# TritonDataCenter/node-cueball

Hardware: AMD Instinct MI355X
Metric: pool claims/sec (8-backend synthetic TCP set) (higher is better)
Workload: dtype n/a; 1 GPU; model=ConnectionPool claim/release (config: headline), global_batch=20000, seq_len=1, parallelism=1 worker processes (event loops), backends=8, spares=8, maximum=16, concurrency=16

## Files before the change

cueball_amd/_native/speed.cpp:

```cpp

#define PY_SSIZE_T_CLEAN
#include <Python.h>
#include <structmember.h>
#include <cmath>
#include <cstring>
#include <ctime>

#include "lathist.h"

#ifndef CUEBALL_HANDLE_HOOKS
#define CUEBALL_HANDLE_HOOKS 1
#endif
#ifndef CUEBALL_SLOT_HOOKS
#define CUEBALL_SLOT_HOOKS 1
#endif
#ifndef CUEBALL_LAZY_SCOPES
#define CUEBALL_LAZY_SCOPES 1
#endif
#ifndef CUEBALL_VECTORCALL
#define CUEBALL_VECTORCALL 1
#endif
#ifndef CUEBALL_EXACT_TYPES
#define CUEBALL_EXACT_TYPES 1
#endif
#ifndef CUEBALL_VALID_IDENTITY
#define CUEBALL_VALID_IDENTITY 1
#endif
#if !defined(Py_TPFLAGS_HAVE_VECTORCALL) && defined(_Py_TPFLAGS_HAVE_VECTORCALL)
#define Py_TPFLAGS_HAVE_VECTORCALL _Py_TPFLAGS_HAVE_VECTORCALL
#endif

namespace {

PyObject *s_stateChanged;
PyObject *s_listener;
PyObject *s_on;
PyObject *s_remove_listener;
PyObject *s_call_soon;
PyObject *s_call_later;
PyObject *s_cancel;
PyObject *s_state_prefix;
PyObject *s_dot;
PyObject *s_underscore;
PyObject *s_flush_name;
PyObject *s_internal;
PyObject *s_is_closed;

PyObject *g_get_loop;
PyObject *g_fsm_error;
PyObject *g_entry_name_cache;
PyObject *g_flush_batches;
PyObject *g_tracer;
PyObject *g_remove_desc;

static inline PyObject *
resolve_loop(PyObject *loop)
{
    if (loop != NULL && loop != Py_None) {
        Py_INCREF(loop);
        return loop;
    }
    return PyObject_CallOneArg(g_get_loop, Py_None);
}


typedef struct {
    PyObject_HEAD
    PyObject *ev_events;
    PyObject *ev_dict;
    PyObject *ev_weakrefs;
    unsigned long ev_gen;
    unsigned long ev_lk_gen;
    long ev_lk_cnt[4];
    Py_ssize_t ev_lk_len[4];
    int ev_lk_ok;
} Emitter;

extern PyTypeObject EmitterType;
extern PyTypeObject ConnErrCbType;
extern PyTypeObject KitCbType;

static inline int
listener_is_own_internal(PyObject *listener)
{
    PyTypeObject *tp = Py_TYPE(listener);
    return tp == &ConnErrCbType || tp == &KitCbType;
}

#define SMALL_LIST_KEEP 8

static inline int
list_append_keep(PyObject *ls, PyObject *item)
{
    PyListObject *l = (PyListObject *)ls;
    Py_ssize_t n = Py_SIZE(l);
    if (n < l->allocated) {
        Py_INCREF(item);
        l->ob_item[n] = item;
        Py_SET_SIZE(l, n + 1);
        return 0;
    }
    return PyList_Append(ls, item);
}

static inline int
list_remove_at_keep(PyObject *ls, Py_ssize_t i)
{
    PyListObject *l = (PyListObject *)ls;
    Py_ssize_t n = Py_SIZE(l);
    if (l->allocated > SMALL_LIST_KEEP)
        return PyList_SetSlice(ls, i, i + 1, NULL);
    PyObject *item = l->ob_item[i];
    for (Py_ssize_t j = i; j + 1 < n; j++)
        l->ob_item[j] = l->ob_item[j + 1];
    Py_SET_SIZE(l, n - 1);
    Py_DECREF(item);
    return 0;
}

int
Emitter_init(PyObject *self_, PyObject *args, PyObject *kwds)
{
    Emitter *self = (Emitter *)self_;
    (void)args; (void)kwds;
    if (self->ev_events == NULL) {
        self->ev_events = PyDict_New();
        if (self->ev_events == NULL)
            return -1;
    }
    return 0;
}

int
Emitter_traverse(PyObject *self_, visitproc visit, void *arg)
{
    Emitter *self = (Emitter *)self_;
    Py_VISIT(self->ev_events);
    Py_VISIT(self->ev_dict);
    return 0;
}

int
Emitter_clear_(PyObject *self_)
{
    Emitter *self = (Emitter *)self_;
    Py_CLEAR(self->ev_events);
    Py_CLEAR(self->ev_dict);
    return 0;
}

void
Emitter_dealloc(PyObject *self_)
{
    Emitter *self = (Emitter *)self_;
    PyTypeObject *tp = Py_TYPE(self_);
    PyObject_GC_UnTrack(self_);
    if (self->ev_weakrefs != NULL)
        PyObject_ClearWeakRefs(self_);
    Emitter_clear_(self_);
    tp->tp_free(self_);
}

PyObject *
emitter_add(Emitter *self, PyObject *event, PyObject *listener)
{
    if (self->ev_events == NULL) {
        self->ev_events = PyDict_New();
        if (self->ev_events == NULL)
            return NULL;
    }
    PyObject *ls = PyDict_GetItemWithError(self->ev_events, event);
    if (ls == NULL) {
        if (PyErr_Occurred())
            return NULL;
        ls = PyList_New(0);
        if (ls == NULL)
            return NULL;
        if (PyDict_SetItem(self->ev_events, event, ls) < 0) {
            Py_DECREF(ls);
            return NULL;
        }
        Py_DECREF(ls);
    }
    if (list_append_keep(ls, listener) < 0)
        return NULL;
    if (!listener_is_own_internal(listener))
        self->ev_gen++;
    Py_INCREF(listener);
    return listener;
}

PyObject *
Emitter_on(PyObject *self_, PyObject *const *args, Py_ssize_t nargs)
{
    if (nargs != 2) {
        PyErr_SetString(PyExc_TypeError, "on(event, listener)");
        return NULL;
    }
    return emitter_add((Emitter *)self_, args[0], args[1]);
}

typedef struct {
    PyObject_HEAD
    PyObject *ow_emitter;
    PyObject *ow_event;
    PyObject *ow_listener;
} OnceWrapper;

extern PyTypeObject OnceWrapperType;

PyObject *
OnceWrapper_call(PyObject *self_, PyObject *args, PyObject *kwds)
{
    OnceWrapper *self = (OnceWrapper *)self_;
    (void)kwds;
    PyObject *res = PyObject_CallMethodObjArgs(
        self->ow_emitter, s_remove_listener, self->ow_event,
        (PyObject *)self, NULL);
    if (res == NULL)
        return NULL;
    Py_DECREF(res);
    return PyObject_Call(self->ow_listener, args, NULL);
}

PyObject *
OnceWrapper_get_listener(PyObject *self_, void *closure)
{
    OnceWrapper *self = (OnceWrapper *)self_;
// ... 694 lines not shown
    return 0;
}

int
Scope_clear_(PyObject *self_)
{
    Scope *self = (Scope *)self_;
    Py_CLEAR(self->sc_fsm);
    Py_CLEAR(self->sc_listeners);
    Py_CLEAR(self->sc_timers);
    int nreg = self->sc_nreg;
    self->sc_nreg = 0;
    for (int i = 0; i < 3 * nreg; i++)
        Py_CLEAR(self->sc_reg[i]);
    return 0;
}

void
Scope_dealloc(PyObject *self_)
{
    PyObject_GC_UnTrack(self_);
    Scope_clear_(self_);
    if (scope_freelist_n < SCOPE_FREELIST_MAX)
        scope_freelist[scope_freelist_n++] = (Scope *)self_;
    else
        PyObject_GC_Del(self_);
}

PyMethodDef Scope_methods[] = {
    {"on", (PyCFunction)(void (*)(void))Scope_on, METH_FASTCALL, NULL},
    {"timeout", (PyCFunction)(void (*)(void))Scope_timeout, METH_FASTCALL,
     NULL},
    {"interval", (PyCFunction)(void (*)(void))Scope_interval,
     METH_FASTCALL, NULL},
    {"immediate", Scope_immediate, METH_O, NULL},
    {"callback", Scope_callback, METH_O, NULL},
    {"valid_transitions", Scope_valid_transitions, METH_O, NULL},
    {"goto_state", Scope_goto_state, METH_O, NULL},
    {"_dispose", Scope_dispose, METH_NOARGS, NULL},
    {NULL, NULL, 0, NULL},
};

PyGetSetDef Scope_getset[] = {
    {(char *)"active", Scope_get_active, NULL, NULL, NULL},
    {NULL, NULL, NULL, NULL, NULL},
};

PyTypeObject ScopeType = {
    PyVarObject_HEAD_INIT(NULL, 0)
    "cueball_amd._speed.StateScope",
    sizeof(Scope),
    0,
    Scope_dealloc,
    0, 0, 0, 0, 0, 0, 0, 0, 0, 0, 0, 0, 0, 0,
    Py_TPFLAGS_DEFAULT | Py_TPFLAGS_HAVE_GC,
    "FSM state scope (native)",
    Scope_traverse,
    Scope_clear_,
    0, 0, 0, 0,
    Scope_methods,
    0,
    Scope_getset,
};


struct FSMOb {
    Emitter base;
    PyObject *f_loop;
    PyObject *f_state;
    PyObject *f_scope;
    PyObject *f_valid;
    PyObject *f_pending;
    PyObject **f_eq;
    Py_ssize_t f_eq_head, f_eq_len, f_eq_cap;
    PyObject *f_eq_inl[4];
    PyObject *f_hist[8];
    unsigned long f_hist_n;
    PyObject *f_flush_bound;
    PyObject *f_fastkit;
    PyObject *f_watchkit;
    PyObject *f_ctx;
    int f_entering;
    int f_emit_scheduled;
};

int slotkit_maybe_entry(PyObject *kit_, FSMOb *fsm, PyObject *target);
int slotkit_smgr_hook(PyObject *kit_, PyObject *st, unsigned long serial);
unsigned long slotkit_slot_serial(PyObject *kit_);
int ch_emit_state_changed(FSMOb *self, PyObject *st);

static inline Scope *
fsm_need_scope(FSMOb *self)
{
    if (self->f_scope == NULL)
        self->f_scope = (PyObject *)scope_new((PyObject *)self);
    return (Scope *)self->f_scope;
}

extern PyObject *t_empty;
extern PyTypeObject CHType;
extern PyTypeObject CTType;
void ch_terminal_cleanup(FSMOb *self);

typedef PyObject *(*ch_entry_fn)(PyObject *, PyObject *);
ch_entry_fn ch_direct_entry(FSMOb *self, PyObject *target);

extern PyTypeObject FSMType;
extern PyTypeObject SlotBaseType;

PyTypeObject *g_handle_cls;
PyTypeObject *g_slot_cls;
PyTypeObject *g_pool_cls;

static inline int
is_handle(PyObject *x)
{
#if CUEBALL_EXACT_TYPES
    if (Py_TYPE(x) == g_handle_cls)
        return 1;
#endif
    return PyObject_TypeCheck(x, &CHType);
}

static inline int
is_slot(PyObject *x)
{
#if CUEBALL_EXACT_TYPES
    if (Py_TYPE(x) == g_slot_cls)
        return 1;
#endif
    return PyObject_TypeCheck(x, &SlotBaseType);
}

static inline int
is_fsm(PyObject *x)
{
#if CUEBALL_EXACT_TYPES
    PyTypeObject *tp = Py_TYPE(x);
    if (tp == g_pool_cls || tp == g_slot_cls || tp == g_handle_cls)
        return 1;
#endif
    return PyObject_TypeCheck(x, &FSMType);
}

PyObject *
fsm_get_loop_of(FSMOb *fsm)
{
    return fsm->f_loop;
}

#define FSM_EQ_INLINE 4
#define FSM_HISTORY 8

static void
fsm_eq_compact(FSMOb *f)
{
    if (f->f_eq_head == 0)
        return;
    Py_ssize_t n = f->f_eq_len - f->f_eq_head;
    memmove(f->f_eq, f->f_eq + f->f_eq_head, n * sizeof(PyObject *));
    f->f_eq_head = 0;
    f->f_eq_len = n;
}

static int
fsm_eq_push(FSMOb *f, PyObject *st)
{
    if (f->f_eq == NULL) {
        f->f_eq = f->f_eq_inl;
        f->f_eq_cap = FSM_EQ_INLINE;
        f->f_eq_head = f->f_eq_len = 0;
    }
    if (f->f_eq_len == f->f_eq_cap) {
        if (f->f_eq_head > 0) {
            fsm_eq_compact(f);
        } else {
            Py_ssize_t ncap = f->f_eq_cap * 2;
            PyObject **items;
            if (f->f_eq == f->f_eq_inl) {
                items = (PyObject **)PyMem_Malloc(
                    ncap * sizeof(PyObject *));
                if (items != NULL)
                    memcpy(items, f->f_eq_inl, sizeof(f->f_eq_inl));
            } else {
                items = (PyObject **)PyMem_Realloc(
// ... 234 lines not shown
            Py_DECREF(fb);
            return -1;
        }
        Py_DECREF(h);
        batch = (PyObject *)fb;
        Py_DECREF(fb);
    }
    if (PyList_Append(((FlushBatch *)batch)->fb_list,
                      (PyObject *)self) < 0)
        return -1;
    return 0;
}

PyObject *
entry_attr_name(PyObject *state)
{
    PyObject *name = PyDict_GetItemWithError(g_entry_name_cache, state);
    if (name != NULL) {
        Py_INCREF(name);
        return name;
    }
    if (PyErr_Occurred())
        return NULL;
    PyObject *replaced = PyObject_CallMethod(state, "replace", "OO",
                                             s_dot, s_underscore);
    if (replaced == NULL)
        return NULL;
    name = PyUnicode_Concat(s_state_prefix, replaced);
    Py_DECREF(replaced);
    if (name == NULL)
        return NULL;
    PyUnicode_InternInPlace(&name);
    if (PyDict_SetItem(g_entry_name_cache, state, name) < 0) {
        Py_DECREF(name);
        return NULL;
    }
    return name;
}

int
check_valid(FSMOb *self, PyObject *from, PyObject *state)
{
    if (self->f_valid == NULL)
        return 0;
#if CUEBALL_VALID_IDENTITY
    if (PyTuple_CheckExact(self->f_valid)) {
        PyObject *v = self->f_valid;
        for (Py_ssize_t i = 0, n = PyTuple_GET_SIZE(v); i < n; i++)
            if (PyTuple_GET_ITEM(v, i) == state)
                return 0;
    }
#endif
    int c = PySequence_Contains(self->f_valid, state);
    if (c < 0)
        return -1;
    if (!c) {
        PyErr_Format(g_fsm_error,
                     "%s: invalid transition %R -> %R (valid: %R)",
                     Py_TYPE(self)->tp_name,
                     from ? from : Py_None, state, self->f_valid);
        return -1;
    }
    return 0;
}

int
fsm_enter_loop(FSMOb *self, PyObject *state)
{
    PyObject *next_state = state;
    Py_INCREF(next_state);
    while (next_state != NULL) {
        PyObject *target = next_state;
        next_state = NULL;
        if (self->f_scope != NULL) {
            PyObject *old = self->f_scope;
            self->f_scope = NULL;
            PyObject *r = Scope_dispose(old, NULL);
            Py_DECREF(old);
            if (r == NULL) {
                Py_DECREF(target);
                return -1;
            }
            Py_DECREF(r);
        }
        Py_CLEAR(self->f_valid);
        Py_INCREF(target);
        Py_XSETREF(self->f_state, target);
        Py_INCREF(target);
        Py_XSETREF(self->f_hist[self->f_hist_n % FSM_HISTORY], target);
        self->f_hist_n++;
#if !CUEBALL_LAZY_SCOPES
        if (fsm_need_scope(self) == NULL) {
            Py_DECREF(target);
            return -1;
        }
#endif

        if (g_tracer != NULL && g_tracer != Py_None) {
            PyObject *targs[2] = {(PyObject *)self, target};
            PyObject *tr = PyObject_Vectorcall(g_tracer, targs, 2, NULL);
            if (tr == NULL) {
                Py_DECREF(target);
                return -1;
            }
            Py_DECREF(tr);
        }

        int handled = 0;
        if (self->f_fastkit != NULL) {
            self->f_entering = 1;
            handled = slotkit_maybe_entry(self->f_fastkit, self, target);
            self->f_entering = 0;
            if (handled < 0) {
                Py_DECREF(target);
                return -1;
            }
        }
        PyObject *r;
        ch_entry_fn direct = handled ? NULL : ch_direct_entry(self, target);
        if (handled) {
            r = Py_None;
            Py_INCREF(r);
        } else if (direct != NULL) {
            self->f_entering = 1;
            r = direct((PyObject *)self, NULL);
            self->f_entering = 0;
        } else {
            PyObject *attr = entry_attr_name(target);
            if (attr == NULL) {
                Py_DECREF(target);
                return -1;
            }
            PyObject *entry = PyObject_GetAttr((PyObject *)self, attr);
            Py_DECREF(attr);
            if (entry == NULL) {
                PyErr_Clear();
                PyErr_Format(g_fsm_error,
                             "%s has no state-entry function for %R",
                             Py_TYPE(self)->tp_name, target);
                Py_DECREF(target);
                return -1;
            }
            PyObject *scope = (PyObject *)fsm_need_scope(self);
            if (scope == NULL) {
                Py_DECREF(entry);
                Py_DECREF(target);
                return -1;
            }
            Py_INCREF(scope);
            self->f_entering = 1;
            r = PyObject_CallOneArg(entry, scope);
            Py_DECREF(entry);
            Py_DECREF(scope);
            self->f_entering = 0;
        }
        PyObject *pend = self->f_pending;
        self->f_pending = NULL;
        if (r == NULL) {
            Py_XDECREF(pend);
            Py_DECREF(target);
            return -1;
        }
        Py_DECREF(r);
        if (fsm_queue_state_changed(self, target) < 0) {
            Py_XDECREF(pend);
            Py_DECREF(target);
// ... 901 lines not shown
};

static void
latency_types_init(void)
{
    LatHistType.tp_flags = Py_TPFLAGS_DEFAULT;
    LatHistType.tp_methods = LatHist_methods;
    LatHistType.tp_getset = LatHist_getset;
    LatHistType.tp_new = LatHist_new;

    PoolLatType.tp_dealloc = PoolLat_dealloc;
    PoolLatType.tp_flags = Py_TPFLAGS_DEFAULT | Py_TPFLAGS_HAVE_GC;
    PoolLatType.tp_traverse = PoolLat_traverse;
    PoolLatType.tp_clear = PoolLat_clear_;
    PoolLatType.tp_members = PoolLat_members;
    PoolLatType.tp_new = PoolLat_new;
}


PyObject *g_err_claim_timeout;
PyObject *g_err_cueball;
PyObject *g_err_misused;
PyObject *g_capture_stack;

PyObject *s_claim;
PyObject *s_warn;
PyObject *s_incr;
PyObject *s_claim_timeout_evt;
PyObject *s_is_in_state;
PyObject *s_time;
PyObject *s_waiting, *s_claiming, *s_claimed, *s_released, *s_closed,
         *s_cancelled, *s_failed, *s_idle, *s_error_evt;
PyObject *t_waiting_valid;
PyObject *t_claiming_valid;
PyObject *t_claimed_valid;
PyObject *t_empty;
PyObject *s_leak_events[4];

int g_stack_on = 1;
PyObject *g_stack_placeholder;
PyObject *g_inf;

static inline PyObject *
capture_stack(void)
{
    if (!g_stack_on && g_stack_placeholder != NULL) {
        Py_INCREF(g_stack_placeholder);
        return g_stack_placeholder;
    }
    return PyObject_CallNoArgs(g_capture_stack);
}

extern PyObject *s_busy_st;
PyObject *slotkit_conn_err_cb(PyObject *slot, PyObject *handle);

struct NQueue;
typedef struct {
    PyObject_HEAD
    struct NQueue *pc_idleq;
    struct NQueue *pc_waiters;
    struct NQueue *pc_initq;
    PyObject *pc_counters;
    PyObject *pc_dead;
    PoolLatOb *pc_lat;
    PyObject *pc_log;
    int pc_no_codel;
} PoolCtx;

extern PyTypeObject PoolCtxType;
PoolCtx *pool_ctx(PyObject *pool);
PoolCtx *pool_ctx_private(PoolCtx *base, PoolLatOb *lat, PyObject *log);

typedef struct {
    FSMOb base;
    PyObject *chb_pool;
    PyObject *chb_claim_stack;
    PyObject *chb_callback;
    PyObject *chb_slot;
    PyObject *chb_release_stack;
    PyObject *chb_connection;
    PyObject *chb_last_error;
    PyObject *chb_waiter_node;
    PoolCtx *chb_ctx;
    double chb_claim_timeout;
    double chb_started;
    double chb_claimed_at;
    int chb_pre[4];
    unsigned char chb_have_pre;
    unsigned char chb_throw_error;
    unsigned char chb_cancelled;
    unsigned char chb_leak_check;
    unsigned char chb_pinger;
    unsigned char chb_lat_open;
    unsigned char chb_tk_on;
    unsigned char chb_tk_err_on_empty;
    unsigned long chb_bk_serial;
    Py_ssize_t chb_bk_pos;
} CHOb;

extern PyTypeObject CHType;

static inline PoolLatOb *
ch_lat(CHOb *h)
{
    return h->chb_ctx != NULL ? h->chb_ctx->pc_lat : NULL;
}

static inline PyObject *
ch_log(CHOb *h)
{
    return h->chb_ctx != NULL && h->chb_ctx->pc_log != NULL
        ? h->chb_ctx->pc_log : Py_None;
}

long
c_count_listeners(PyObject *emitter, PyObject *event)
{
    if (!PyObject_TypeCheck(emitter, &EmitterType))
        return -2;
    Emitter *em = (Emitter *)emitter;
    if (em->ev_events == NULL)
        return 0;
    PyObject *ls = PyDict_GetItemWithError(em->ev_events, event);
    if (ls == NULL)
        return PyErr_Occurred() ? -1 : 0;
    long count = 0;
    Py_ssize_t n = PyList_GET_SIZE(ls);
    for (Py_ssize_t i = 0; i < n; i++) {
        PyObject *h = PyList_GET_ITEM(ls, i);
        if (!PyCallable_Check(h))
            continue;
        PyObject *marker = NULL;
        if (_PyObject_LookupAttr(h, s_internal, &marker) < 0)
            return -1;
        if (marker != NULL) {
            int truthy = PyObject_IsTrue(marker);
            Py_DECREF(marker);
            if (truthy < 0)
                return -1;
            if (truthy)
                continue;
        }
        PyObject *target = NULL;
        if (Py_TYPE(h) == &OnceWrapperType) {
            target = ((OnceWrapper *)h)->ow_listener;
            Py_INCREF(target);
        } else if (_PyObject_LookupAttr(h, s_listener, &target) < 0) {
            return -1;
        }
        if (target != NULL && target != h) {
            if (_PyObject_LookupAttr(target, s_internal, &marker) < 0) {
                Py_DECREF(target);
                return -1;
            }
            if (marker != NULL) {
                int truthy = PyObject_IsTrue(marker);
                Py_DECREF(marker);
                if (truthy < 0) {
                    Py_DECREF(target);
                    return -1;
                }
                if (truthy) {
                    Py_DECREF(target);
                    continue;
                }
            }
        }
        Py_XDECREF(target);
        count++;
    }
    return count;
}

int
emitter_leak_counts(PyObject *conn, long out[4])
{
    if (!PyObject_TypeCheck(conn, &EmitterType))
        return -2;
    Emitter *em = (Emitter *)conn;
    Py_ssize_t lens[4];
    for (int i = 0; i < 4; i++) {
        PyObject *ls = NULL;
        if (em->ev_events != NULL) {
            ls = PyDict_GetItemWithError(em->ev_events, s_leak_events[i]);
            if (ls == NULL && PyErr_Occurred())
                return -1;
        }
        lens[i] = (ls != NULL && PyList_Check(ls)) ? PyList_GET_SIZE(ls)
                                                   : -1;
    }
    if (em->ev_lk_ok && em->ev_lk_gen == em->ev_gen &&
        memcmp(lens, em->ev_lk_len, sizeof(lens)) == 0) {
        memcpy(out, em->ev_lk_cnt, sizeof(em->ev_lk_cnt));
        return 0;
    }
    unsigned long gen = em->ev_gen;
    for (int i = 0; i < 4; i++) {
        long c = c_count_listeners(conn, s_leak_events[i]);
        if (c < 0)
            return -1;
        out[i] = c;
    }
    em->ev_lk_ok = 0;
    if (gen == em->ev_gen) {
        memcpy(em->ev_lk_cnt, out, sizeof(em->ev_lk_cnt));
        memcpy(em->ev_lk_len, lens, sizeof(lens));
        em->ev_lk_gen = gen;
        em->ev_lk_ok = 1;
    }
    return 0;
}

typedef struct {
    PyObject_HEAD
    PyObject *ce_handle;
} ConnErrCb;

extern PyTypeObject ConnErrCbType;

PyObject *conn_err_fire(CHOb *h, PyObject *err);

PyObject *
ConnErrCb_call(PyObject *self_, PyObject *args, PyObject *kwds)
{
    CHOb *h = (CHOb *)((ConnErrCb *)self_)->ce_handle;
    (void)kwds;
    PyObject *err = (PyTuple_GET_SIZE(args) > 0)
        ? PyTuple_GET_ITEM(args, 0) : Py_None;
    return conn_err_fire(h, err);
}

PyObject *
conn_err_fire(CHOb *h, PyObject *err)
{
    long cnt = c_count_listeners(h->chb_connection, s_error_evt);
    if (cnt == -1)
        return NULL;
    if (cnt == 0 && h->chb_throw_error) {
        if (PyExceptionInstance_Check(err)) {
            PyErr_SetObject((PyObject *)Py_TYPE(err), err);
        } else {
            PyErr_SetObject(PyExc_RuntimeError, err);
        }
        return NULL;
    }
    PyObject *msg = PyUnicode_FromString(
        "connection emitted error while claimed");
    if (msg == NULL)
        return NULL;
    PyObject *r = PyObject_CallMethodObjArgs(ch_log(h), s_warn, msg,
                                             NULL);
    Py_DECREF(msg);
    if (r == NULL)
        return NULL;
    Py_DECREF(r);
    PyObject *evt = PyUnicode_FromString("error-while-claimed");
    if (evt == NULL)
        return NULL;
    r = PyObject_CallMethodObjArgs(h->chb_pool, s_incr, evt, NULL);
    Py_DECREF(evt);
    if (r == NULL)
        return NULL;
    Py_DECREF(r);
    Py_RETURN_NONE;
}

int
ConnErrCb_traverse(PyObject *self_, visitproc visit, void *arg)
{
    Py_VISIT(((ConnErrCb *)self_)->ce_handle);
    return 0;
}

int
ConnErrCb_clear_(PyObject *self_)
{
    Py_CLEAR(((ConnErrCb *)self_)->ce_handle);
    return 0;
}

void
ConnErrCb_dealloc(PyObject *self_)
{
    PyObject_GC_UnTrack(self_);
    ConnErrCb_clear_(self_);
    PyObject_GC_Del(self_);
}

PyObject *
ConnErrCb_get_internal(PyObject *self_, void *closure)
{
    (void)self_; (void)closure;
    Py_RETURN_TRUE;
// ... 290 lines not shown
        if (cb == NULL) {
            Py_DECREF(ms);
            return NULL;
        }
        PyObject *args[2] = {ms, cb};
        PyObject *r = Scope_timeout(scope, args, 2);
        Py_DECREF(ms);
        Py_DECREF(cb);
        if (r == NULL)
            return NULL;
        Py_DECREF(r);
    }
    Py_RETURN_NONE;
}

PyObject *
CH_state_claiming(PyObject *self_, PyObject *scope)
{
    CHOb *self = (CHOb *)self_;
    (void)scope;
    Py_INCREF(t_claiming_valid);
    Py_XSETREF(self->base.f_valid, t_claiming_valid);
    PyObject *slot = self->chb_slot;
    if (slot != NULL && is_slot(slot) &&
        ((FSMOb *)slot)->f_fastkit != NULL) {
        FSMOb *sf = (FSMOb *)slot;
        PyObject *fs = sf->f_state;
        if (!(fs == s_idle ||
              (fs != NULL && PyUnicode_Compare(fs, s_idle) == 0))) {
            PyErr_SetString(g_fsm_error, "claim only in idle");
            return NULL;
        }
        if (slot_field_set(&((SlotOb *)slot)->sl_handle)) {
            PyErr_SetString(g_fsm_error, "slot already has a handle");
            return NULL;
        }
        slot_field_store(&((SlotOb *)slot)->sl_handle, self_);
        if (fsm_goto_state(sf, s_busy_st) < 0)
            return NULL;
        Py_RETURN_NONE;
    }
    PyObject *r = PyObject_CallMethodObjArgs(slot, s_claim,
                                             self_, NULL);
    if (r == NULL)
        return NULL;
    Py_DECREF(r);
    Py_RETURN_NONE;
}

PyObject *
CH_state_claimed(PyObject *self_, PyObject *scope)
{
    CHOb *self = (CHOb *)self_;
    Py_INCREF(t_claimed_valid);
    Py_XSETREF(self->base.f_valid, t_claimed_valid);

    if (self->chb_cancelled) {
        if (fsm_goto_state(&self->base, s_released) < 0)
            return NULL;
        Py_RETURN_NONE;
    }

    PyObject *conn = self->chb_connection;
    long pre[4] = {0, 0, 0, 0};
    int lk = emitter_leak_counts(conn, pre);
    if (lk == -1)
        return NULL;
    for (int i = 0; i < 4; i++)
        self->chb_pre[i] = lk == -2 ? 0 : (int)pre[i];
    self->chb_have_pre = 1;

    PyObject *ec = slotkit_conn_err_cb(self->chb_slot, self_);
    if (ec != NULL) {
        Py_INCREF(ec);
    } else {
        ConnErrCb *nec = PyObject_GC_New(ConnErrCb, &ConnErrCbType);
        if (nec == NULL)
            return NULL;
        Py_INCREF(self_);
        nec->ce_handle = self_;
        PyObject_GC_Track((PyObject *)nec);
        ec = (PyObject *)nec;
    }
    if (scope == NULL)
        scope = (PyObject *)fsm_need_scope(&self->base);
    if (scope == NULL) {
        Py_DECREF(ec);
        return NULL;
    }
    PyObject *args[3] = {conn, s_error_evt, ec};
    PyObject *r = Scope_on(scope, args, 3);
    Py_DECREF(ec);
    if (r == NULL)
        return NULL;
    Py_DECREF(r);

    PoolLatOb *lat = ch_lat(self);
    if (lat != NULL && !self->chb_pinger) {
        int err = 0;
        double now = poollat_now_ms(lat, &err);
        if (err)
            return NULL;
        lat->pl_wait->h.record_ms(now - self->chb_started);
        self->chb_claimed_at = now;
        self->chb_lat_open = 1;
    }

    PyObject *cbargs[3] = {Py_None, self_, conn};
    r = PyObject_Vectorcall(self->chb_callback, cbargs, 3, NULL);
    if (r == NULL)
        return NULL;
    Py_DECREF(r);
    Py_RETURN_NONE;
}

static int
ch_record_hold(CHOb *self)
{
    if (!self->chb_lat_open)
        return 0;
    self->chb_lat_open = 0;
    PoolLatOb *lat = ch_lat(self);
    if (lat == NULL)
        return 0;
    int err = 0;
    double now = poollat_now_ms(lat, &err);
    if (err)
        return -1;
    lat->pl_hold->h.record_ms(now - self->chb_claimed_at);
    return 0;
}

PyObject *
CH_state_released(PyObject *self_, PyObject *scope)
{
    CHOb *self = (CHOb *)self_;
    (void)scope;
    Py_INCREF(t_empty);
    Py_XSETREF(self->base.f_valid, t_empty);
    if (ch_record_hold(self) < 0)
        return NULL;
    if (!self->chb_leak_check || !self->chb_have_pre)
        Py_RETURN_NONE;
    PyObject *conn = self->chb_connection;
    long after[4];
    int lk = emitter_leak_counts(conn, after);
    if (lk == -1)
        return NULL;
    if (lk == -2)
        Py_RETURN_NONE;
    for (int i = 0; i < 4; i++) {
        long c = after[i];
        if (c > (long)self->chb_pre[i]) {
            PyObject *msg = PyUnicode_FromFormat(
                "connection claimer looks like it leaked event handlers "
                "(event=%S before=%ld after=%ld)",
                s_leak_events[i], (long)self->chb_pre[i], c);
            if (msg == NULL)
                return NULL;
            PyObject *r = PyObject_CallMethodObjArgs(ch_log(self), s_warn,
                                                     msg, NULL);
            Py_DECREF(msg);
            if (r == NULL)
                return NULL;
            Py_DECREF(r);
        }
    }
    Py_RETURN_NONE;
}

PyObject *
CH_state_closed(PyObject *self_, PyObject *scope)
{
    CHOb *self = (CHOb *)self_;
    (void)scope;
    Py_INCREF(t_empty);
    Py_XSETREF(self->base.f_valid, t_empty);
    if (ch_record_hold(self) < 0)
        return NULL;
    Py_RETURN_NONE;
}

PyObject *
CH_state_cancelled(PyObject *self_, PyObject *scope)
{
    CHOb *self = (CHOb *)self_;
    (void)scope;
    Py_INCREF(t_empty);
    Py_XSETREF(self->base.f_valid, t_empty);
    Py_RETURN_NONE;
}

PyObject *
CH_state_failed(PyObject *self_, PyObject *scope)
{
    CHOb *self = (CHOb *)self_;
// ... 24 lines not shown
    PyObject *err = PyObject_CallNoArgs(g_err_misused);
    if (err == NULL)
        return NULL;
    PyErr_SetObject(g_err_misused, err);
    Py_DECREF(err);
    return NULL;
}

PyObject *
CH_on(PyObject *self_, PyObject *const *args, Py_ssize_t nargs)
{
    if (nargs >= 1 && PyUnicode_Check(args[0])) {
        if (PyUnicode_CompareWithASCIIString(args[0], "readable") == 0 ||
            PyUnicode_CompareWithASCIIString(args[0], "close") == 0) {
            PyObject *err = PyObject_CallNoArgs(g_err_misused);
            if (err == NULL)
                return NULL;
            PyErr_SetObject(g_err_misused, err);
            Py_DECREF(err);
            return NULL;
        }
    }
    return Emitter_on(self_, args, nargs);
}

PyObject *
CH_once(PyObject *self_, PyObject *const *args, Py_ssize_t nargs)
{
    if (nargs >= 1 && PyUnicode_Check(args[0])) {
        if (PyUnicode_CompareWithASCIIString(args[0], "readable") == 0 ||
            PyUnicode_CompareWithASCIIString(args[0], "close") == 0) {
            PyObject *err = PyObject_CallNoArgs(g_err_misused);
            if (err == NULL)
                return NULL;
            PyErr_SetObject(g_err_misused, err);
            Py_DECREF(err);
            return NULL;
        }
    }
    return Emitter_once(self_, args, nargs);
}

PyObject *
CH_remove_listener(PyObject *self_, PyObject *const *args, Py_ssize_t nargs)
{
    CHOb *self = (CHOb *)self_;
    if (nargs != 2) {
        PyErr_SetString(PyExc_TypeError, "remove_listener(event, listener)");
        return NULL;
    }
    Py_ssize_t at;
    if (emitter_remove_core(&self->base.base, args, &at) < 0)
        return NULL;
    if (at >= 0 && at < self->chb_bk_pos &&
        (args[0] == s_stateChanged ||
         (PyUnicode_Check(args[0]) &&
          PyUnicode_Compare(args[0], s_stateChanged) == 0)))
        self->chb_bk_pos--;
    Py_RETURN_NONE;
}

PyObject *
CH_remove_all_listeners(PyObject *self_, PyObject *const *args,
                        Py_ssize_t nargs)
{
    ((CHOb *)self_)->chb_bk_pos = 0;
    return Emitter_remove_all_listeners(self_, args, nargs);
}


int
CH_traverse(PyObject *self_, visitproc visit, void *arg)
{
    CHOb *self = (CHOb *)self_;
    Py_VISIT(self->chb_pool);
    Py_VISIT(self->chb_claim_stack);
    Py_VISIT(self->chb_callback);
    Py_VISIT(self->chb_slot);
    Py_VISIT(self->chb_release_stack);
    Py_VISIT(self->chb_connection);
    Py_VISIT(self->chb_last_error);
    Py_VISIT(self->chb_waiter_node);
    Py_VISIT((PyObject *)self->chb_ctx);
    return FSM_traverse(self_, visit, arg);
}

int
CH_clear_(PyObject *self_)
{
    CHOb *self = (CHOb *)self_;
    Py_CLEAR(self->chb_pool);
    Py_CLEAR(self->chb_claim_stack);
    Py_CLEAR(self->chb_callback);
    Py_CLEAR(self->chb_slot);
    Py_CLEAR(self->chb_release_stack);
    Py_CLEAR(self->chb_connection);
    Py_CLEAR(self->chb_last_error);
    Py_CLEAR(self->chb_waiter_node);
    Py_CLEAR(self->chb_ctx);
    return FSM_clear_(self_);
}

void
CH_dealloc(PyObject *self_)
{
    CHOb *self = (CHOb *)self_;
    PyTypeObject *tp = Py_TYPE(self_);
    PyObject_GC_UnTrack(self_);
    if (self->base.base.ev_weakrefs != NULL)
        PyObject_ClearWeakRefs(self_);
    CH_clear_(self_);
    tp->tp_free(self_);
}

PyObject *
CH__setup(PyObject *self_, PyObject *const *args, Py_ssize_t nargs)
{
    CHOb *self = (CHOb *)self_;
    if (nargs != 7) {
        PyErr_SetString(PyExc_TypeError,
            "_setup(pool, stack, cb, log, timeout, throw_error, loop)");
        return NULL;
    }
    Py_INCREF(args[0]); Py_XSETREF(self->chb_pool, args[0]);
    Py_INCREF(args[1]); Py_XSETREF(self->chb_claim_stack, args[1]);
    Py_INCREF(args[2]); Py_XSETREF(self->chb_callback, args[2]);
    self->chb_claim_timeout = PyFloat_AsDouble(args[4]);
    if (self->chb_claim_timeout == -1.0 && PyErr_Occurred())
        return NULL;
    int throw_error = PyObject_IsTrue(args[5]);
    if (throw_error < 0)
        return NULL;
    self->chb_throw_error = throw_error;
    self->chb_cancelled = 0;
    self->chb_leak_check = 1;
    self->chb_pinger = 0;
    self->chb_have_pre = 0;
    self->chb_lat_open = 0;
    PoolCtx *cx = pool_ctx(args[0]);
    if (cx != NULL && cx->pc_log == args[3]) {
        Py_INCREF((PyObject *)cx);
    } else {
        PyObject *lat = NULL;
        if (cx != NULL) {
            lat = (PyObject *)cx->pc_lat;
            Py_XINCREF(lat);
        } else {
            if (_PyObject_LookupAttr(args[0], s_p_lat, &lat) < 0)
                return NULL;
            if (lat != NULL && Py_TYPE(lat) != &PoolLatType)
                Py_CLEAR(lat);
        }
        cx = pool_ctx_private(cx, (PoolLatOb *)lat, args[3]);
        Py_XDECREF(lat);
        if (cx == NULL)
            return NULL;
    }
    Py_XSETREF(self->chb_ctx, cx);

    PyObject *resolved = resolve_loop(args[6]);
    if (resolved == NULL)
        return NULL;
    Py_XSETREF(self->base.f_loop, resolved);
#if !CUEBALL_HANDLE_HOOKS
    if (Emitter_init(self_, NULL, NULL) < 0)
        return NULL;
#endif
    self->chb_tk_on = 0;
    self->chb_bk_serial = 0;
    if (fsm_goto_state(&self->base, s_waiting) < 0)
        return NULL;
    PoolLatOb *plat = ch_lat(self);
    if (plat != NULL && plat->pl_direct &&
        plat->pl_loop == self->base.f_loop) {
        int err = 0;
        self->chb_started = poollat_now_ms(plat, &err);
        if (err)
            return NULL;
        Py_RETURN_NONE;
    }
    PyObject *t = PyObject_CallMethodObjArgs(self->base.f_loop, s_time,
                                             NULL);
// ... 2743 lines not shown
static void
claim_method_type_init(void)
{
    ClaimMethodType.tp_dealloc = ClaimMethod_dealloc;
    ClaimMethodType.tp_vectorcall_offset =
        offsetof(ClaimMethod, cm_vectorcall);
    ClaimMethodType.tp_call = PyVectorcall_Call;
    ClaimMethodType.tp_flags = Py_TPFLAGS_DEFAULT | Py_TPFLAGS_HAVE_GC |
        Py_TPFLAGS_HAVE_VECTORCALL | Py_TPFLAGS_METHOD_DESCRIPTOR;
    ClaimMethodType.tp_traverse = ClaimMethod_traverse;
    ClaimMethodType.tp_clear = ClaimMethod_clear_;
    ClaimMethodType.tp_members = ClaimMethod_members;
    ClaimMethodType.tp_descr_get = ClaimMethod_descr_get;
}

static PyObject *
speed_claim_method(PyObject *mod, PyObject *const *args, Py_ssize_t nargs)
{
    (void)mod;
    if (nargs != 2 || !PyCallable_Check(args[0]) || !PyType_Check(args[1]) ||
        !PyType_IsSubtype((PyTypeObject *)args[1], &CHType)) {
        PyErr_SetString(PyExc_TypeError,
                        "claim_method(func, ClaimHandleBase subclass)");
        return NULL;
    }
#if !CUEBALL_VECTORCALL
    Py_INCREF(args[0]);
    return args[0];
#else
    ClaimMethod *cm = PyObject_GC_New(ClaimMethod, &ClaimMethodType);
    if (cm == NULL)
        return NULL;
    Py_INCREF(args[0]);
    cm->cm_func = args[0];
    Py_INCREF(args[1]);
    cm->cm_handle_cls = args[1];
    cm->cm_vectorcall = ClaimMethod_vectorcall;
    cm->cm_doc = PyObject_GetAttrString(args[0], "__doc__");
    cm->cm_name = PyObject_GetAttrString(args[0], "__name__");
    cm->cm_qualname = PyObject_GetAttrString(args[0], "__qualname__");
    cm->cm_module = PyObject_GetAttrString(args[0], "__module__");
    PyErr_Clear();
    PyObject_GC_Track((PyObject *)cm);
    return (PyObject *)cm;
#endif
}

static PyObject *
speed_set_cycle_classes(PyObject *mod, PyObject *const *args,
                        Py_ssize_t nargs)
{
    (void)mod;
    if (nargs != 3) {
        PyErr_SetString(PyExc_TypeError,
                        "_set_cycle_classes(handle_cls, slot_cls, pool_cls)");
        return NULL;
    }
    PyTypeObject *bases[3] = {&CHType, &SlotBaseType, &FSMType};
    PyTypeObject **dst[3] = {&g_handle_cls, &g_slot_cls, &g_pool_cls};
    for (int i = 0; i < 3; i++) {
        if (args[i] == Py_None)
            continue;
        PyTypeObject *cls = (PyTypeObject *)args[i];
        if (!PyType_Check(args[i]) || !PyType_IsSubtype(cls, bases[i]) ||
            (i > 0 && PyType_IsSubtype(cls, &CHType)) ||
            (i == 2 && PyType_IsSubtype(cls, &SlotBaseType))) {
            PyErr_SetString(PyExc_TypeError,
                "_set_cycle_classes: a ClaimHandleBase, a SlotBase and a "
                "plain FSM subclass required");
            return NULL;
        }
    }
    for (int i = 0; i < 3; i++) {
        if (args[i] == Py_None)
            continue;
        Py_INCREF(args[i]);
        PyTypeObject *old = *dst[i];
        *dst[i] = (PyTypeObject *)args[i];
        Py_XDECREF((PyObject *)old);
    }
    Py_RETURN_NONE;
}

PyObject *
speed_set_tracer(PyObject *mod, PyObject *fn)
{
    (void)mod;
    if (fn == Py_None) {
        Py_CLEAR(g_tracer);
    } else {
        Py_INCREF(fn);
        Py_XSETREF(g_tracer, fn);
    }
    Py_RETURN_NONE;
}

PyMethodDef speed_methods[] = {
    {"_set_claim_helpers",
     (PyCFunction)(void (*)(void))speed_set_claim_helpers, METH_FASTCALL,
     NULL},
    {"_set_tracer", speed_set_tracer, METH_O, NULL},
    {"_set_stack_traces",
     (PyCFunction)(void (*)(void))speed_set_stack_traces, METH_FASTCALL,
     NULL},
    {"count_listeners",
     (PyCFunction)(void (*)(void))speed_count_listeners, METH_FASTCALL,
     NULL},
    {"_set_helpers", (PyCFunction)(void (*)(void))speed_set_helpers,
     METH_FASTCALL, NULL},
    {"claim_fast", (PyCFunction)(void (*)(void))speed_claim_fast,
     METH_FASTCALL, NULL},
    {"pool_claim", (PyCFunction)(void (*)(void))speed_pool_claim,
     METH_FASTCALL, NULL},
    {"claim_method", (PyCFunction)(void (*)(void))speed_claim_method,
     METH_FASTCALL, NULL},
    {"_set_cycle_classes",
     (PyCFunction)(void (*)(void))speed_set_cycle_classes, METH_FASTCALL,
     NULL},
    {NULL, NULL, 0, NULL},
};

struct PyModuleDef speedmodule = {
    PyModuleDef_HEAD_INIT,
    "cueball_amd._speed",
    "Native event/FSM runtime core",
    -1,
    speed_methods,
};

}

PyMODINIT_FUNC
PyInit__speed(void)
{
    s_stateChanged = PyUnicode_InternFromString("stateChanged");
    s_listener = PyUnicode_InternFromString("listener");
    s_on = PyUnicode_InternFromString("on");
    s_remove_listener = PyUnicode_InternFromString("remove_listener");
    s_call_soon = PyUnicode_InternFromString("call_soon");
    s_call_later = PyUnicode_InternFromString("call_later");
    s_cancel = PyUnicode_InternFromString("cancel");
    s_state_prefix = PyUnicode_InternFromString("state_");
    s_dot = PyUnicode_InternFromString(".");
    s_underscore = PyUnicode_InternFromString("_");
    s_flush_name = PyUnicode_InternFromString("_flush_state_changed");
    s_internal = PyUnicode_InternFromString("_cueball_internal");
    s_is_closed = PyUnicode_InternFromString("is_closed");
    s_claim = PyUnicode_InternFromString("claim");
    s_warn = PyUnicode_InternFromString("warn");
    s_incr = PyUnicode_InternFromString("_incr_counter");
    s_claim_timeout_evt = PyUnicode_InternFromString("claim-timeout");
    s_is_in_state = PyUnicode_InternFromString("is_in_state");
    s_time = PyUnicode_InternFromString("time");
    s_waiting = PyUnicode_InternFromString("waiting");
    s_claiming = PyUnicode_InternFromString("claiming");
    s_claimed = PyUnicode_InternFromString("claimed");
    s_released = PyUnicode_InternFromString("released");
    s_closed = PyUnicode_InternFromString("closed");
    s_cancelled = PyUnicode_InternFromString("cancelled");
    s_failed = PyUnicode_InternFromString("failed");
    s_idle = PyUnicode_InternFromString("idle");
    s_error_evt = PyUnicode_InternFromString("error");
    t_waiting_valid = PyTuple_Pack(3, s_claiming, s_cancelled, s_failed);
    t_claiming_valid = PyTuple_Pack(3, s_claimed, s_waiting, s_cancelled);
    t_claimed_valid = PyTuple_Pack(2, s_released, s_closed);
    t_empty = PyTuple_New(0);
    s_leak_events[0] = PyUnicode_InternFromString("close");
    s_leak_events[1] = s_error_evt;
    s_leak_events[2] = PyUnicode_InternFromString("readable");
    s_leak_events[3] = PyUnicode_InternFromString("data");
    g_entry_name_cache = PyDict_New();
    if (g_entry_name_cache == NULL)
        return NULL;
    g_flush_batches = PyDict_New();
    if (g_flush_batches == NULL)
        return NULL;

    s_running_st = PyUnicode_InternFromString("running");
    s_p_idleq_node = PyUnicode_InternFromString("p_idleq_node");
    s_p_total_conns = PyUnicode_InternFromString("p_total_conns");
    s_p_busy_hwm = PyUnicode_InternFromString("p_busy_hwm");
    s_p_demand_hwm = PyUnicode_InternFromString("p_demand_hwm");
    s_ticket_slow = PyUnicode_InternFromString("_ticket_slow");
    s_p_idleq = PyUnicode_InternFromString("p_idleq");
    s_p_waiters = PyUnicode_InternFromString("p_waiters");
    s_p_initq = PyUnicode_InternFromString("p_initq");
    s_p_counters = PyUnicode_InternFromString("p_counters");
    s_p_rebal_scheduled = PyUnicode_InternFromString("p_rebal_scheduled");
    s_max_claim_queue = PyUnicode_InternFromString("max-claim-queue");
    s_queued_claim = PyUnicode_InternFromString("queued-claim");
    s_connected_st = PyUnicode_InternFromString("connected");
    s_busy_st = PyUnicode_InternFromString("busy");
    s_stopping_st = PyUnicode_InternFromString("stopping");
    s_stopped_st = PyUnicode_InternFromString("stopped");
    s_retrying_st = PyUnicode_InternFromString("retrying");
    s_connecting_st = PyUnicode_InternFromString("connecting");
    s_killing_st = PyUnicode_InternFromString("killing");
    s_unwanted_evt = PyUnicode_InternFromString("unwanted");
    s_sm_socket = PyUnicode_InternFromString("sm_socket");
    t_busy_valid = PyTuple_Pack(6, s_idle, s_stopping_st, s_stopped_st,
// ... 96 lines not shown
```

Baseline: 871,300 claims/s.

## Cache leak-listener counts by dict version tag and register conn error handler directly

Moves the per-emitter leak-count cache into a separately allocated struct that also holds the listener lists and the events dict's version tag. This lets a cache hit skip the four dict lookups when the dict is unchanged. Separately, the claim handle registers its connection 'error' listener directly on the connection instead of lazily creating a Scope, and unregisters it on the next state transition. The aim is to avoid scope allocation and disposal per claim, at the cost of more complex lifetime bookkeeping and a dependency on a dict internal field that is disabled on Python 3.12+.

```diff
diff --git a/cueball_amd/_native/speed.cpp b/cueball_amd/_native/speed.cpp
--- a/cueball_amd/_native/speed.cpp
+++ b/cueball_amd/_native/speed.cpp
@@ -8,6 +8,16 @@
 
 #include "lathist.h"
 
+#ifndef CUEBALL_LEAK_TAG
+#define CUEBALL_LEAK_TAG 1
+#endif
+#ifndef CUEBALL_OWN_CONN_ERR
+#define CUEBALL_OWN_CONN_ERR 1
+#endif
+#if CUEBALL_LEAK_TAG && PY_VERSION_HEX >= 0x030C0000
+#undef CUEBALL_LEAK_TAG
+#define CUEBALL_LEAK_TAG 0
+#endif
 #ifndef CUEBALL_HANDLE_HOOKS
 #define CUEBALL_HANDLE_HOOKS 1
 #endif
@@ -70,11 +80,17 @@
     PyObject *ev_dict;
     PyObject *ev_weakrefs;
     unsigned long ev_gen;
-    unsigned long ev_lk_gen;
-    long ev_lk_cnt[4];
-    Py_ssize_t ev_lk_len[4];
-    int ev_lk_ok;
+    struct LeakCache *ev_lk;
 } Emitter;
+
+struct LeakCache {
+    int lk_ok;
+    unsigned long lk_gen;
+    long lk_cnt[4];
+    Py_ssize_t lk_len[4];
+    uint64_t lk_ver;
+    PyObject *lk_list[4];
+};
 
 extern PyTypeObject EmitterType;
 extern PyTypeObject ConnErrCbType;
@@ -137,13 +153,34 @@
     Emitter *self = (Emitter *)self_;
     Py_VISIT(self->ev_events);
     Py_VISIT(self->ev_dict);
+    if (self->ev_lk != NULL)
+        for (int i = 0; i < 4; i++)
+            Py_VISIT(self->ev_lk->lk_list[i]);
     return 0;
+}
+
+static void
+emitter_lk_drop(Emitter *self)
+{
+    LeakCache *lk = self->ev_lk;
+    if (lk == NULL)
+        return;
+    lk->lk_ok = 0;
+    for (int i = 0; i < 4; i++)
+        Py_CLEAR(lk->lk_list[i]);
 }
 
 int
 Emitter_clear_(PyObject *self_)
 {
     Emitter *self = (Emitter *)self_;
+    LeakCache *lk = self->ev_lk;
+    if (lk != NULL) {
+        self->ev_lk = NULL;
+        for (int i = 0; i < 4; i++)
+            Py_CLEAR(lk->lk_list[i]);
+        PyMem_Free(lk);
+    }
     Py_CLEAR(self->ev_events);
     Py_CLEAR(self->ev_dict);
     return 0;
@@ -1004,6 +1041,7 @@
     PyObject *f_ctx;
     int f_entering;
     int f_emit_scheduled;
+    int f_own_reg;
 };
 
 int slotkit_maybe_entry(PyObject *kit_, FSMOb *fsm, PyObject *target);
@@ -1023,6 +1061,7 @@
 extern PyTypeObject CHType;
 extern PyTypeObject CTType;
 void ch_terminal_cleanup(FSMOb *self);
+int ch_drop_conn_err(FSMOb *self);
 
 typedef PyObject *(*ch_entry_fn)(PyObject *, PyObject *);
 ch_entry_fn ch_direct_entry(FSMOb *self, PyObject *target);
@@ -1423,6 +1462,10 @@
                 return -1;
             }
             Py_DECREF(r);
+        }
+        if (self->f_own_reg && ch_drop_conn_err(self) < 0) {
+            Py_DECREF(target);
+            return -1;
         }
         Py_CLEAR(self->f_valid);
         Py_INCREF(target);
@@ -2490,6 +2533,8 @@
     PyObject *chb_last_error;
     PyObject *chb_waiter_node;
     PoolCtx *chb_ctx;
+    PyObject *chb_err_conn;
+    PyObject *chb_err_cb;
     double chb_claim_timeout;
     double chb_started;
     double chb_claimed_at;
@@ -2580,13 +2625,40 @@
     return count;
 }
 
+static inline Py_ssize_t
+leak_list_len(PyObject *ls)
+{
+    return (ls != NULL && PyList_Check(ls)) ? PyList_GET_SIZE(ls) : -1;
+}
+
 int
 emitter_leak_counts(PyObject *conn, long out[4])
 {
     if (!PyObject_TypeCheck(conn, &EmitterType))
         return -2;
     Emitter *em = (Emitter *)conn;
+    LeakCache *lk = em->ev_lk;
+#if CUEBALL_LEAK_TAG
+    if (lk != NULL && lk->lk_ok && lk->lk_gen == em->ev_gen &&
+        em->ev_events != NULL &&
+        lk->lk_ver == ((PyDictObject *)em->ev_events)->ma_version_tag) {
+        int same = 1;
+        for (int i = 0; i < 4; i++) {
+            same &= (leak_list_len(lk->lk_list[i]) == lk->lk_len[i]);
+        }
+        if (same) {
+            memcpy(out, lk->lk_cnt, sizeof(lk->lk_cnt));
+            return 0;
+        }
+    }
+#endif
     Py_ssize_t lens[4];
+    PyObject *lists[4];
+    uint64_t ver = 0;
+#if CUEBALL_LEAK_TAG
+    if (em->ev_events != NULL)
+        ver = ((PyDictObject *)em->ev_events)->ma_version_tag;
+#endif
     for (int i = 0; i < 4; i++) {
         PyObject *ls = NULL;
         if (em->ev_events != NULL) {
@@ -2594,29 +2666,48 @@
             if (ls == NULL && PyErr_Occurred())
                 return -1;
         }
-        lens[i] = (ls != NULL && PyList_Check(ls)) ? PyList_GET_SIZE(ls)
-                                                   : -1;
-    }
-    if (em->ev_lk_ok && em->ev_lk_gen == em->ev_gen &&
-        memcmp(lens, em->ev_lk_len, sizeof(lens)) == 0) {
-        memcpy(out, em->ev_lk_cnt, sizeof(em->ev_lk_cnt));
+        lists[i] = ls;
+        lens[i] = leak_list_len(ls);
+    }
+    lk = em->ev_lk;
+    if (lk != NULL && lk->lk_ok && lk->lk_gen == em->ev_gen &&
+        memcmp(lens, lk->lk_len, sizeof(lens)) == 0 &&
+        memcmp(lists, lk->lk_list, sizeof(lists)) == 0) {
+        lk->lk_ver = ver;
+        memcpy(out, lk->lk_cnt, sizeof(lk->lk_cnt));
         return 0;
     }
     unsigned long gen = em->ev_gen;
-    for (int i = 0; i < 4; i++) {
+    for (int i = 0; i < 4; i++)
+        Py_XINCREF(lists[i]);
+    int failed = 0;
+    for (int i = 0; i < 4 && !failed; i++) {
         long c = c_count_listeners(conn, s_leak_events[i]);
         if (c < 0)
-            return -1;
+            failed = 1;
         out[i] = c;
     }
-    em->ev_lk_ok = 0;
-    if (gen == em->ev_gen) {
-        memcpy(em->ev_lk_cnt, out, sizeof(em->ev_lk_cnt));
-        memcpy(em->ev_lk_len, lens, sizeof(lens));
-        em->ev_lk_gen = gen;
-        em->ev_lk_ok = 1;
-    }
-    return 0;
+    emitter_lk_drop(em);
+    lk = em->ev_lk;
+    if (!failed && lk == NULL && em->ev_events != NULL) {
+        lk = (LeakCache *)PyMem_Calloc(1, sizeof(LeakCache));
+        em->ev_lk = lk;
+    }
+    if (!failed && lk != NULL && !lk->lk_ok && gen == em->ev_gen &&
+        em->ev_events != NULL) {
+        memcpy(lk->lk_cnt, out, sizeof(lk->lk_cnt));
+        memcpy(lk->lk_len, lens, sizeof(lens));
+        for (int i = 0; i < 4; i++) {
+            Py_XSETREF(lk->lk_list[i], lists[i]);
+            lists[i] = NULL;
+        }
+        lk->lk_ver = ver;
+        lk->lk_gen = gen;
+        lk->lk_ok = 1;
+    }
+    for (int i = 0; i < 4; i++)
+        Py_XDECREF(lists[i]);
+    return failed ? -1 : 0;
 }
 
 typedef struct {
@@ -3073,18 +3164,39 @@
         PyObject_GC_Track((PyObject *)nec);
         ec = (PyObject *)nec;
     }
-    if (scope == NULL)
-        scope = (PyObject *)fsm_need_scope(&self->base);
-    if (scope == NULL) {
+    PyObject *r;
+#if CUEBALL_OWN_CONN_ERR
+    if (scope == NULL && !self->base.f_own_reg) {
+        if (Py_TYPE(conn) == &EmitterType)
+            r = emitter_add((Emitter *)conn, s_error_evt, ec);
+        else
+            r = PyObject_CallMethodObjArgs(conn, s_on, s_error_evt, ec,
+                                           NULL);
+        if (r == NULL) {
+            Py_DECREF(ec);
+            return NULL;
+        }
+        Py_DECREF(r);
+        Py_INCREF(conn);
+        self->chb_err_conn = conn;
+        self->chb_err_cb = ec;
+        self->base.f_own_reg = 1;
+    } else
+#endif
+    {
+        if (scope == NULL)
+            scope = (PyObject *)fsm_need_scope(&self->base);
+        if (scope == NULL) {
+            Py_DECREF(ec);
+            return NULL;
+        }
+        PyObject *args[3] = {conn, s_error_evt, ec};
+        r = Scope_on(scope, args, 3);
         Py_DECREF(ec);
-        return NULL;
-    }
-    PyObject *args[3] = {conn, s_error_evt, ec};
-    PyObject *r = Scope_on(scope, args, 3);
-    Py_DECREF(ec);
-    if (r == NULL)
-        return NULL;
-    Py_DECREF(r);
+        if (r == NULL)
+            return NULL;
+        Py_DECREF(r);
+    }
 
     PoolLatOb *lat = ch_lat(self);
     if (lat != NULL && !self->chb_pinger) {
@@ -3103,6 +3215,24 @@
         return NULL;
     Py_DECREF(r);
     Py_RETURN_NONE;
+}
+
+int
+ch_drop_conn_err(FSMOb *fsm)
+{
+    CHOb *self = (CHOb *)fsm;
+    PyObject *conn = self->chb_err_conn, *cb = self->chb_err_cb;
+    self->chb_err_conn = self->chb_err_cb = NULL;
+    fsm->f_own_reg = 0;
+    if (conn == NULL || cb == NULL) {
+        Py_XDECREF(conn);
+        Py_XDECREF(cb);
+        return 0;
+    }
+    int rc = scope_unregister(conn, s_error_evt, cb);
+    Py_DECREF(conn);
+    Py_DECREF(cb);
+    return rc;
 }
 
 static int
@@ -3293,6 +3423,8 @@
     Py_VISIT(self->chb_last_error);
     Py_VISIT(self->chb_waiter_node);
     Py_VISIT((PyObject *)self->chb_ctx);
+    Py_VISIT(self->chb_err_conn);
+    Py_VISIT(self->chb_err_cb);
     return FSM_traverse(self_, visit, arg);
 }
 
@@ -3309,6 +3441,9 @@
     Py_CLEAR(self->chb_last_error);
     Py_CLEAR(self->chb_waiter_node);
     Py_CLEAR(self->chb_ctx);
+    self->base.f_own_reg = 0;
+    Py_CLEAR(self->chb_err_conn);
+    Py_CLEAR(self->chb_err_cb);
     return FSM_clear_(self_);
 }
 
@@ -6218,6 +6353,30 @@
     Py_RETURN_NONE;
 }
 
+static PyObject *
+speed_debug_cycle_state(PyObject *mod, PyObject *const *args,
+                        Py_ssize_t nargs)
+{
+    (void)mod;
+    PyObject *lk = Py_None;
+    Py_INCREF(lk);
+    if (nargs >= 1 && PyObject_TypeCheck(args[0], &EmitterType)) {
+        LeakCache *c = ((Emitter *)args[0])->ev_lk;
+        if (c != NULL && c->lk_ok &&
+            c->lk_gen == ((Emitter *)args[0])->ev_gen) {
+            Py_DECREF(lk);
+            lk = Py_BuildValue("(llll)", c->lk_cnt[0], c->lk_cnt[1],
+                               c->lk_cnt[2], c->lk_cnt[3]);
+            if (lk == NULL)
+                return NULL;
+        }
+    }
+    return Py_BuildValue("{s:N,s:i,s:i}",
+                         "leak_cache", lk,
+                         "leak_tag", (int)CUEBALL_LEAK_TAG,
+                         "own_conn_err", (int)CUEBALL_OWN_CONN_ERR);
+}
+
 PyObject *
 speed_set_tracer(PyObject *mod, PyObject *fn)
 {
@@ -6252,6 +6411,9 @@
      METH_FASTCALL, NULL},
     {"_set_cycle_classes",
      (PyCFunction)(void (*)(void))speed_set_cycle_classes, METH_FASTCALL,
+     NULL},
+    {"_debug_cycle_state",
+     (PyCFunction)(void (*)(void))speed_debug_cycle_state, METH_FASTCALL,
      NULL},
     {NULL, NULL, 0, NULL},
 };
```

New measurement: 918,100 claims/s (median of 6 runs). 5.4% higher.
